# michellelychan/posenet-pytorch

Measured on NVIDIA B200. Metric: images/sec (backbone+decode), higher is better.
Workload: dtype bf16

## Files before the change

posenet-pytorch_b200/csrc/sepconv.cu:

```cuda
#include <cuda.h>
#include <stdlib.h>
#include <string.h>

#include "common.cuh"
#include "ptx.cuh"

namespace pn {

#ifndef PN_SEP_DW_WARPS
#define PN_SEP_DW_WARPS 10
#endif
constexpr int SEP_DW_WARPS = PN_SEP_DW_WARPS;
constexpr int SEP_FIRST_DW_WARP = 6;
constexpr int SEP_THREADS = (SEP_FIRST_DW_WARP + SEP_DW_WARPS) * 32;
constexpr int SEP_MAX_A = 6;
constexpr int SEP_A_BYTES = 128 * 128;
constexpr int SEP_STG_BYTES = 128 * 128;
constexpr int SEP_MAX_P = 6, SEP_MAX_W = 6;
constexpr int SEP_WGT_BYTES = 9 * 64 * 4 + 64 * 4;
constexpr int SEP_SMEM_MAX = 232448;
constexpr int SEP_DWW_KB_BYTES = 10 * 64 * 4;

struct SepGeom {
    int k, nc, ho, wo, pad;
    int th, tw, subs, ths, thi, twi;
    int spr, seg_rows, segs_per_sub;
    unsigned segtab[64];
    int tiles_x, tiles_y, n_tiles, n_tile, panels, tmem_cols;
    int n_halves, n_half, acc_bufs;
    int kblocks;
    int half, cbox;
    int cl;
    int dww_res;
    int w_res;
    unsigned off_dww;
    int teams;
    int exp;
    unsigned epi_sleep_ns;
    int p_stages, w_stages, a_stages, stg_bufs;
    unsigned patch_stage_bytes, patch_box_bytes, wgt_off, w_stage_bytes;
    unsigned off_a, off_stg, off_patch, off_bias, off_bar;
    long long tiles;
};

struct SepBars {
    static constexpr int patch_full = 0, patch_empty = 8 * SEP_MAX_P, w_full = 16 * SEP_MAX_P,
                         w_empty = 16 * SEP_MAX_P + 8 * SEP_MAX_W, a_full = 16 * SEP_MAX_P + 16 * SEP_MAX_W,
                         a_empty = a_full + 8 * SEP_MAX_A, tfull = a_empty + 8 * SEP_MAX_A, tempty = tfull + 16,
                         tmem_slot = tempty + 16, seg_ctr = tmem_slot + 16, seg_tab = seg_ctr + 4 * 8, total = seg_tab + 4 * 64;
};

__device__ __forceinline__ uint64_t sep_smem_desc(uint32_t saddr) {
    return (uint64_t)((saddr & 0x3FFFF) >> 4) | (1ull << 16) | ((uint64_t)(1024 >> 4) << 32) | (1ull << 46) | (2ull << 61);
}
__device__ __forceinline__ uint32_t sep_idesc(int n) {
    return (1u << 4) | (1u << 7) | (1u << 10) | ((uint32_t)(n >> 3) << 17) | ((uint32_t)(128 >> 4) << 24);
}
__device__ __forceinline__ void sep_epi_bar() { asm volatile("bar.sync 1, 128;" ::: "memory"); }
__device__ __forceinline__ float4 lds_f4(uint32_t addr) {
    float4 r;
    asm volatile("ld.shared.v4.f32 {%0, %1, %2, %3}, [%4];" : "=f"(r.x), "=f"(r.y), "=f"(r.z), "=f"(r.w) : "r"(addr));
    return r;
}
__device__ __forceinline__ bool mbar_test(uint32_t bar, uint32_t parity) {
    uint32_t done;
    asm volatile("{\n\t.reg .pred p;\n\tmbarrier.test_wait.parity.shared::cta.b64 p, [%1], %2;\n\tselp.u32 %0, 1, 0, p;\n\t}"
                 : "=r"(done) : "r"(bar), "r"(parity) : "memory");
    return done != 0;
}
__device__ __forceinline__ float2 lds_f2(uint32_t addr) {
    float2 r;
    asm volatile("ld.shared.v2.f32 {%0, %1}, [%2];" : "=f"(r.x), "=f"(r.y) : "r"(addr));
    return r;
}
__device__ __forceinline__ uint32_t lds_u32(uint32_t addr) {
    uint32_t r;
    asm volatile("ld.shared.b32 %0, [%1];" : "=r"(r) : "r"(addr));
    return r;
}
__device__ __forceinline__ uint32_t cluster_rank() {
    uint32_t r;
    asm volatile("mov.u32 %0, %%cluster_ctarank;" : "=r"(r));
    return r;
}
__device__ __forceinline__ void cluster_sync_all() {
    asm volatile("barrier.cluster.arrive.release.aligned;" ::: "memory");
    asm volatile("barrier.cluster.wait.acquire.aligned;" ::: "memory");
}
__device__ __forceinline__ uint32_t map_to_cta(uint32_t saddr, uint32_t rank) {
    uint32_t r;
    asm volatile("mapa.shared::cluster.u32 %0, %1, %2;" : "=r"(r) : "r"(saddr), "r"(rank));
    return r;
}
__device__ __forceinline__ void remote_expect_tx(uint32_t cluster_bar, uint32_t bytes) {
    asm volatile("mbarrier.arrive.expect_tx.release.cluster.shared::cluster.b64 _, [%0], %1;" ::"r"(cluster_bar), "r"(bytes) : "memory");
}
__device__ __forceinline__ void dsmem_bulk_copy(uint32_t cluster_dst, uint32_t src, uint32_t bytes, uint32_t cluster_bar) {
    asm volatile("cp.async.bulk.shared::cluster.shared::cta.mbarrier::complete_tx::bytes [%0], [%1], %2, [%3];" ::"r"(cluster_dst),
                 "r"(src), "r"(bytes), "r"(cluster_bar)
                 : "memory");
}
__device__ __forceinline__ void tc_commit_multicast(uint32_t bar, uint16_t cta_mask) {
    asm volatile("tcgen05.commit.cta_group::1.mbarrier::arrive::one.shared::cluster.multicast::cluster.b64 [%0], %1;" ::"r"(bar),
                 "h"(cta_mask)
                 : "memory");
}
__device__ __forceinline__ void sts_u32_if(uint32_t addr, uint32_t v, bool on) {
    if (on) asm volatile("st.shared.b32 [%0], %1;" ::"r"(addr), "r"(v) : "memory");
}

template <int S, int D, bool HALF> struct SepDwCfg {
    static constexpr bool SLIDE = true;
    static constexpr int RSTEP = (S == 1) ? D : 1;
    static constexpr int DR = (S == 1) ? 1 : D;
    static constexpr bool UNPACKED = (D <= 2);
    static constexpr int NR = 2 * DR + 1;
    static constexpr int HS = HALF ? 2 * S : S;
    static constexpr int NCOLS = 3 * HS + 2 * D + 1;
    static constexpr int PRE = 2 * DR + 1 - S;
};


#ifdef PN_SEP_TRACE
__device__ long long *g_sep_trace = nullptr;
__device__ int g_sep_trace_cap = 0;
#endif
#if defined(PN_SEP_TRACE) && !defined(PN_SEP_PHASES)
#define SEP_TRACE(role, idx, what)                                                                               \
    do {                                                                                                         \
        if (blockIdx.x == 0 && g_sep_trace && (idx) < g_sep_trace_cap)                                           \
            g_sep_trace[((role) * g_sep_trace_cap + (idx)) * 4 + (what)] = clock64();                            \
    } while (0)
#else
#define SEP_TRACE(role, idx, what) do { } while (0)
#endif

// ... 73 lines not shown
    if (DWW_RES) {
        float *sw = reinterpret_cast<float *>(sep_smem_raw + (base - smem_u32(sep_smem_raw)) + g.off_dww);
        for (int i = threadIdx.x; i < g.kblocks * 640; i += SEP_THREADS) {
            const int kbi = i / 640, r = i - kbi * 640, t = r >> 6, ch = kbi * 64 + (r & 63);
            sw[i] = ch < g.k ? (t < 9 ? __ldg(dw_w + (size_t)t * g.k + ch) : __ldg(dw_b + ch)) : 0.f;
        }
    }
    tc_fence_before();
    __syncthreads();
    if (CLUSTER) cluster_sync_all();
    tc_fence_after();
    pdl_launch_dependents();
    pdl_wait();
    const uint32_t tmem_base = *tmem_slot_ptr;

    if (warp == 0) {
        if (lane == 0) {
            int ps = 0, ws = 0, tr_p = 0;
            uint32_t pph = 0, wph = 0;
            (void)tr_p;
            long long p_tile = tile_first, w_tile = tile_first;
            int p_kb = rank, p_sub = 0, w_kb = 0, w_hf = 0;
            int p_img = 0, p_ty = 0, p_tx = 0, w_col = 0;
            bool p_new = true, w_new = true;
            int s_as = rank;
            uint32_t s_aph = 0;
            long long s_left = 0;
            if (CLUSTER && tile_first < g.tiles) s_left = ((g.tiles - tile_first + tile_step - 1) / tile_step) * (g.kblocks / CL);
            const long long t0 = clock64();
            while (p_tile < g.tiles || w_tile < g.tiles || s_left > 0) {
                bool progress = false;
                if (CLUSTER && s_left > 0 && mbar_test(bar(SepBars::a_full, s_as), s_aph)) {
                    const uint32_t sa = a_addr(s_as);
#pragma unroll
                    for (int pr = 0; pr < CL; ++pr)
                        if (pr != rank) {
                            const uint32_t rbar = map_to_cta(bar(SepBars::a_full, s_as), (uint32_t)pr);
                            remote_expect_tx(rbar, SEP_A_BYTES);
                            dsmem_bulk_copy(map_to_cta(sa, (uint32_t)pr), sa, SEP_A_BYTES, rbar);
                        }
                    s_as += CL;
                    if (s_as >= g.a_stages) { s_as -= g.a_stages; s_aph ^= 1; }
                    --s_left;
                    progress = true;
                }
                if (p_tile < g.tiles) {
                    if (p_new) {
                        const int m_tile = (int)(p_tile / g.n_tiles);
                        p_img = m_tile / m_tiles_per_img;
                        const int rem = m_tile - p_img * m_tiles_per_img;
                        p_ty = rem / g.tiles_x;
                        p_tx = rem - p_ty * g.tiles_x;
                        p_new = false;
                    }
                    if (mbar_test(bar(SepBars::patch_empty, ps), pph ^ 1)) {
                        const uint32_t full = bar(SepBars::patch_full, ps);
                        SEP_TRACE(3, tr_p, 0);
#ifdef PN_SEP_EXP
                        if (g.exp & 32) mbar_arrive(full); else {
#endif
                        mbar_expect_tx(full, g.patch_box_bytes + (DWW_RES ? 0u : (uint32_t)SEP_WGT_BYTES));
                        tma_load_4d(p_addr(ps), &tmap_x, full, p_kb * CB, p_tx * g.tw * S - g.pad,
                                    (p_ty * g.th + p_sub * g.ths) * S - g.pad, p_img);
                        if (!DWW_RES) {
                            tma_load_2d(p_addr(ps) + g.wgt_off, &tmap_dww, full, p_kb * CB, 0);
                            tma_load_2d(p_addr(ps) + g.wgt_off + 9 * 64 * 4, &tmap_dwb, full, p_kb * CB, 0);
                        }
#ifdef PN_SEP_EXP
                        }
#endif
                        SEP_TRACE(3, tr_p, 1);
                        ++tr_p;
                        if (++ps == g.p_stages) { ps = 0; pph ^= 1; }
                        if (++p_sub == g.subs) {
                            p_sub = 0;
                            p_kb += CL;
                            if (p_kb >= g.kblocks) { p_kb = rank; p_tile += tile_step; p_new = true; }
                        }
                        progress = true;
                    }
                }
                if (w_tile < g.tiles) {
                    if (w_new) { w_col = col_base + (int)(w_tile % g.n_tiles) * g.n_tile; w_new = false; }
                    if (mbar_test(bar(SepBars::w_empty, ws), wph ^ 1)) {
#ifdef PN_SEP_EXP
                        if (g.exp & 8) mbar_arrive(bar(SepBars::w_full, ws)); else {
#endif
                        mbar_expect_tx(bar(SepBars::w_full, ws), g.w_stage_bytes);
                        tma_load_2d(w_addr(ws), &tmap_w, bar(SepBars::w_full, ws), w_kb * CB, w_col + w_hf * g.n_half);
#ifdef PN_SEP_EXP
                        }
#endif
                        if (++ws == g.w_stages) { ws = 0; wph ^= 1; }
                        if (++w_hf == g.n_halves) {
                            w_hf = 0;
                            if (++w_kb == g.kblocks) {
                                w_kb = 0; w_tile += tile_step; w_new = true;
                                if (g.w_res) w_tile = g.tiles;
                            }
                        }
                        progress = true;
                    }
                }
                if (!progress) {
                    __nanosleep(32);
                    if (clock64() - t0 > 20000000000ll) {
                        printf("posenet_b200: sepconv producer timeout (block %d)\n", blockIdx.x);
                        __trap();
                    }
                }
            }
        }
    } else if (warp == 1) {
        if (lane == 0) {
            const uint32_t idesc = sep_idesc(g.n_half);
            int as = 0, ws = 0, acc = 0, tr_i = 0;
            uint32_t aph = 0, wph = 0, acc_phase = 0;
            (void)tr_i;
            long long kb_total = 0;
            for (long long tile = tile_first; tile < g.tiles; tile += tile_step) {
                mbar_wait(bar(SepBars::tempty, acc), acc_phase ^ 1);
                tc_fence_after();
                SEP_TRACE(1, tr_i, 0);
                const uint32_t d_tmem = tmem_base + (uint32_t)(acc * g.n_tile);
                for (int kb = 0; kb < g.kblocks; ++kb) {
                    mbar_wait(bar(SepBars::a_full, as), aph);
                    SEP_TRACE(1, tr_i, 1);
                    const uint32_t sa = a_addr(as);
                    const int rem_k = g.k - kb * CB;
                    const int ksteps = rem_k >= CB ? CB / 16 : (rem_k + 15) / 16;
                    for (int hf = 0; hf < g.n_halves; ++hf) {
                        if (g.w_res) {
                            ws = kb * g.n_halves + hf;
                            if (tile == tile_first) mbar_wait(bar(SepBars::w_full, ws), 0);
                        } else
                            mbar_wait(bar(SepBars::w_full, ws), wph);
                        tc_fence_after();
                        const uint32_t sb = w_addr(ws);
#pragma unroll
                        for (int k = 0; k < CB / 16; ++k)
                            if (k < ksteps
#ifdef PN_SEP_EXP
                                && !(g.exp & 4)
#endif
                                )
                                tc_mma_bf16(d_tmem + (uint32_t)(hf * g.n_half), sep_smem_desc(sa + k * 32), sep_smem_desc(sb + k * 32), idesc,
                                            (uint32_t)((kb | k) != 0));
                        if (!g.w_res) {
                            tc_commit(bar(SepBars::w_empty, ws));
                            if (++ws == g.w_stages) { ws = 0; wph ^= 1; }
                        }
                    }
                    if (CLUSTER) tc_commit_multicast(bar(SepBars::a_empty, as), (uint16_t)((1u << CL) - 1u));
                    else tc_commit(bar(SepBars::a_empty, as));
                    ++kb_total;
                    SEP_TRACE(1, tr_i, 2);
                    ++tr_i;
                    if (++as == g.a_stages) { as = 0; aph ^= 1; }
                }
                tc_commit(bar(SepBars::tfull, acc));
                if (++acc == g.acc_bufs) { acc = 0; acc_phase ^= 1; }
            }
            if (CLUSTER) {
                for (int s2 = 0; s2 < g.a_stages; ++s2) {
                    if (kb_total <= s2) continue;
                    const long long uses = (kb_total - s2 + g.a_stages - 1) / g.a_stages;
                    mbar_wait(bar(SepBars::a_empty, s2), (uint32_t)((uses - 1) & 1));
                }
            }
        }
    } else if (warp < SEP_FIRST_DW_WARP) {
        const int q = warp & 3;
        const int row_in_tile = q * 32 + lane;
        const bool issuer = (threadIdx.x == 64);
        const uint32_t staging = base + g.off_stg;
        int acc = 0, buf = 0, tr_e = 0;
        uint32_t acc_phase = 0;
        (void)tr_e;
        if (g.stg_bufs == 0) {
            const int r_ty = row_in_tile / g.tw, r_tx = row_in_tile - r_ty * g.tw;
            const int chunks = (g.n_tile + 31) >> 5;
            auto emit = [&](const uint32_t (&v)[32], int c, __nv_bfloat16 *yrow, bool row_ok, int col_lim, uint32_t bias_base) {
                const int col0 = c * 32;
#pragma unroll
                for (int piece = 0; piece < 2; ++piece) {
                    uint32_t o[8];
#pragma unroll
                    for (int j = 0; j < 8; j += 2) {
                        const float4 b0 = lds_f4(bias_base + (uint32_t)(col0 + piece * 16 + j * 2) * 4u);
                        const int i0 = piece * 16 + j * 2;
                        const float2 s0 = fadd2(make_float2(__uint_as_float(v[i0 + 0]), __uint_as_float(v[i0 + 1])), make_float2(b0.x, b0.y));
                        const float2 s1 = fadd2(make_float2(__uint_as_float(v[i0 + 2]), __uint_as_float(v[i0 + 3])), make_float2(b0.z, b0.w));
                        o[j] = relu6_bf16x2(s0);
                        o[j + 1] = relu6_bf16x2(s1);
                    }
                    if (row_ok && col0 + piece * 16 < col_lim)
                        asm volatile("st.global.v8.b32 [%0], {%1, %2, %3, %4, %5, %6, %7, %8};" ::"l"(yrow + col0 + piece * 16), "r"(o[0]),
                                     "r"(o[1]), "r"(o[2]), "r"(o[3]), "r"(o[4]), "r"(o[5]), "r"(o[6]), "r"(o[7])
                                     : "memory");
                }
            };
            for (long long tile = tile_first; tile < g.tiles; tile += tile_step) {
                const int n_tile = (int)(tile % g.n_tiles);
                const int m_tile = (int)(tile / g.n_tiles);
                const int img = m_tile / m_tiles_per_img;
                const int rem = m_tile - img * m_tiles_per_img;
                const int ty = rem / g.tiles_x, tx = rem - ty * g.tiles_x;
                const int oy = ty * g.th + r_ty, ox = tx * g.tw + r_tx;
                bool row_ok = r_ty < g.th && oy < g.ho && ox < g.wo;
#ifdef PN_SEP_EXP
                if (g.exp & 16) row_ok = false;
#endif
                const int colg = col_base + n_tile * g.n_tile;
                __nv_bfloat16 *yrow = y + (((size_t)img * g.ho + oy) * g.wo + ox) * (size_t)g.nc + colg;
                const int col_lim = g.nc - colg;
                mbar_wait_backoff(bar(SepBars::tfull, acc), acc_phase, g.epi_sleep_ns);
                tc_fence_after();
                if (issuer) SEP_TRACE(2, tr_e, 0);
                const uint32_t taddr = tmem_base + ((uint32_t)(q * 32) << 16) + (uint32_t)(acc * g.n_tile);
                const uint32_t bias_base = base + g.off_bias + (uint32_t)(n_tile * g.n_tile) * 4u;
                uint32_t va[32], vb[32];
                tc_ld32(taddr, va);
#pragma unroll 1
                for (int c = 0; c < chunks; c += 2) {
                    tc_ld_wait();
                    if (c + 1 < chunks) tc_ld32(taddr + (uint32_t)((c + 1) * 32), vb);
                    else { tc_fence_before(); mbar_arrive(bar(SepBars::tempty, acc)); }
                    emit(va, c, yrow, row_ok, col_lim, bias_base);
                    if (c + 1 < chunks) {
                        tc_ld_wait();
                        if (c + 2 < chunks) tc_ld32(taddr + (uint32_t)((c + 2) * 32), va);
                        else { tc_fence_before(); mbar_arrive(bar(SepBars::tempty, acc)); }
                        emit(vb, c + 1, yrow, row_ok, col_lim, bias_base);
                    }
                }
                if (issuer) { SEP_TRACE(2, tr_e, 1); ++tr_e; }
                if (++acc == g.acc_bufs) { acc = 0; acc_phase ^= 1; }
            }
        } else
        for (long long tile = tile_first; tile < g.tiles; tile += tile_step) {
            const int n_tile = (int)(tile % g.n_tiles);
            const int m_tile = (int)(tile / g.n_tiles);
            const int img = m_tile / m_tiles_per_img;
            const int rem = m_tile - img * m_tiles_per_img;
            const int ty = rem / g.tiles_x, tx = rem - ty * g.tiles_x;
            mbar_wait_backoff(bar(SepBars::tfull, acc), acc_phase, g.epi_sleep_ns);
            tc_fence_after();
            if (issuer) SEP_TRACE(2, tr_e, 0);
            const uint32_t taddr = tmem_base + ((uint32_t)(q * 32) << 16) + (uint32_t)(acc * g.n_tile);
#ifdef PN_SEP_EXP
            if (g.exp & 2) {
                tc_fence_before();
                mbar_arrive(bar(SepBars::tempty, acc));
                if (++acc == g.acc_bufs) { acc = 0; acc_phase ^= 1; }
                continue;
            }
#endif
#pragma unroll 1
            for (int p = 0; p < g.panels; ++p) {
                const int col0 = n_tile * g.n_tile + p * 64;
                if (issuer) {
                    if (g.stg_bufs == 2) bulk_wait_read<1>(); else bulk_wait_read<0>();
                }
                sep_epi_bar();
                const uint32_t srow = staging + (uint32_t)buf * SEP_STG_BYTES + (uint32_t)row_in_tile * 128u;
#pragma unroll
                for (int hf = 0; hf < 2; ++hf) {
                    uint32_t v[32];
                    tc_ld32(taddr + (uint32_t)(p * 64 + hf * 32), v);
                    tc_ld_wait();
                    if (p == g.panels - 1 && hf == 1) {
                        tc_fence_before();
                        mbar_arrive(bar(SepBars::tempty, acc));
                    }
#pragma unroll
                    for (int c = 0; c < 4; ++c) {
                        const uint32_t bsm = base + g.off_bias + (uint32_t)(col0 + hf * 32 + c * 8) * 4u;
                        const float4 b0 = lds_f4(bsm), b1 = lds_f4(bsm + 16);
                        const float2 s0 = fadd2(make_float2(__uint_as_float(v[8 * c + 0]), __uint_as_float(v[8 * c + 1])), make_float2(b0.x, b0.y));
                        const float2 s1 = fadd2(make_float2(__uint_as_float(v[8 * c + 2]), __uint_as_float(v[8 * c + 3])), make_float2(b0.z, b0.w));
                        const float2 s2 = fadd2(make_float2(__uint_as_float(v[8 * c + 4]), __uint_as_float(v[8 * c + 5])), make_float2(b1.x, b1.y));
                        const float2 s3 = fadd2(make_float2(__uint_as_float(v[8 * c + 6]), __uint_as_float(v[8 * c + 7])), make_float2(b1.z, b1.w));
                        st_shared_v4(srow + (uint32_t)(((hf * 4 + c) ^ (row_in_tile & 7)) << 4), relu6_bf16x2(s0), relu6_bf16x2(s1),
                                     relu6_bf16x2(s2), relu6_bf16x2(s3));
                    }
                }
                fence_async_smem();
                sep_epi_bar();
                if (issuer) {
                    tma_store_4d(&tmap_y, staging + (uint32_t)buf * SEP_STG_BYTES, col_base + col0, tx * g.tw, ty * g.th, img);
                    bulk_commit();
                }
                if (g.stg_bufs == 2) buf ^= 1;
            }
            if (issuer) { SEP_TRACE(2, tr_e, 1); ++tr_e; }
            if (++acc == g.acc_bufs) { acc = 0; acc_phase ^= 1; }
        }
        if (issuer) bulk_wait_all();
    } else {
        using Cfg = SepDwCfg<S, D, HALF>;
        constexpr int NR = Cfg::NR, NCOLS = Cfg::NCOLS, PRE = Cfg::PRE, HS = Cfg::HS, RSTEP = Cfg::RSTEP, DR = Cfg::DR;
        constexpr bool SLIDE = Cfg::SLIDE, UNPACKED = Cfg::UNPACKED, PREFETCH = Cfg::UNPACKED;
        constexpr int NNEW = S;
        constexpr uint32_t PIX = HALF ? 64u : 128u;
        const int hsel = HALF ? (lane >> 4) : 0, cp = HALF ? (lane & 15) : lane;
        const uint32_t rowb1 = (uint32_t)g.twi * PIX, rowb = rowb1 * RSTEP;
        const uint32_t lane_off = (uint32_t)(hsel * S) * PIX + (uint32_t)cp * 4u;
        const uint32_t a_lane = (uint32_t)(cp >> 2) << 4 | (uint32_t)(cp & 3) << 2;
        auto unpack = [](uint32_t r) { return make_float2(__uint_as_float(r << 16), __uint_as_float(r & 0xffff0000u)); };
        const uint32_t tab_addr = bars + (uint32_t)SepBars::seg_tab;

        const int n_teams = g.teams, dwi = warp - SEP_FIRST_DW_WARP, team_max = (SEP_DW_WARPS + n_teams - 1) / n_teams;
        const int big_teams = SEP_DW_WARPS - n_teams * (team_max - 1);
        const int team = dwi < big_teams * team_max ? dwi / team_max : big_teams + (dwi - big_teams * team_max) / (team_max - 1);
        const int team_first = team < big_teams ? team * team_max : big_teams * team_max + (team - big_teams) * (team_max - 1);
        const int team_warps = team < big_teams ? team_max : team_max - 1;
        const bool twice = team_warps < team_max && dwi == team_first;
        const int n_subs = g.subs, n_pst = g.p_stages, n_ast = g.a_stages, n_kb = g.kblocks;
        const int item_step = CLUSTER ? CL : n_teams;
        int tr_d = 0;
// ... 185 lines not shown
#include "sep_tuned.inc"
    {0, 0, 0, 0, 0, 0, 0, 0, 0, 0, 0, 0, 0, 0}};
static int next_pow2_cols(int c) {
    int p = 32;
    while (p < c) p <<= 1;
    return p;
}

bool sep_supported(int k, int nc, int stride, int dil) {
    return k % 8 == 0 && nc % 16 == 0 && k >= 8 && nc >= 16 &&
           ((stride == 1 && (dil == 1 || dil == 2 || dil == 4)) || (stride == 2 && dil == 1));
}

bool sep_fuse_recommended(int k, int nc, int stride, int dil) {
    if (!sep_supported(k, nc, stride, dil)) return false;
    if (nc <= 512) return true;
    return nc == 1024 && k % 64 == 0 && (k / 64) % 4 == 0 && getenv("PN_SEP_CLUSTER") != nullptr;
}

int sep_geometry(SepOp *op, int n, int h, int wd, int k, int nc, int stride, int dil) {
    PN_CHECK_ARG(n > 0 && h > 0 && wd > 0, "pn_sepconv_block: bad shape");
    PN_CHECK_ARG(sep_supported(k, nc, stride, dil), "pn_sepconv_block: unsupported block (cin %d cout %d stride %d dilation %d)", k,
                 nc, stride, dil);
    memset(op, 0, sizeof(*op));
    if (sepwarp_supported(k, nc, stride, dil)) {
        op->warp_kind = true;
        op->stride = stride; op->dil = dil;
        op->ho = (h - 1) / stride + 1; op->wo = (wd - 1) / stride + 1;
        op->n = n; op->h = h; op->w = wd; op->k = k; op->nc = nc;
        return PN_OK;
    }
    if (septc_preferred(k, nc, stride, dil)) {
        op->tc_kind = true;
        op->stride = stride; op->dil = dil;
        op->ho = h; op->wo = wd;
        op->n = n; op->h = h; op->w = wd; op->k = k; op->nc = nc;
        return septc_geometry(&op->tc, n, h, wd, k, nc, dil);
    }
    SepGeom g;
    memset(&g, 0, sizeof(g));
    g.k = k; g.nc = nc;
    g.pad = ((stride - 1) + dil * 2) / 2;
    g.ho = (h + 2 * g.pad - 2 * dil - 1) / stride + 1;
    g.wo = (wd + 2 * g.pad - 2 * dil - 1) / stride + 1;
    PN_CHECK_ARG(g.ho > 0 && g.wo > 0, "pn_sepconv_block: empty output");
    const int cb = 64;
    const bool slide = dil == 1;
    g.half = (k <= 32 && stride == 1 && dil == 1) ? 1 : 0;
    g.cbox = g.half ? 32 : cb;
    const int sw = g.half ? 8 : 4;
    const int ncols = 3 * stride * (g.half ? 2 : 1) + 2 * dil + 1, pre = slide ? 2 * dil + 1 - stride : 0;
    g.kblocks = ceil_div(k, cb);
    g.n_tiles = ceil_div(nc, 512);
    g.n_tile = nc / g.n_tiles;
    g.cl = 1;
    if ((nc == 512 || nc == 1024) && k % cb == 0 && (k / cb) % (nc / 256) == 0 && getenv("PN_SEP_CLUSTER") != nullptr) {
        g.cl = nc / 256;
        g.n_tiles = 1;
        g.n_tile = 256;
    }
    g.n_halves = g.n_tile > 256 ? 2 : 1;
    if (const char *e = getenv("PN_SEP_NBLK")) {
        const int want = atoi(e);
        if (want >= 64 && want % 16 == 0 && g.n_tile > want && g.n_tile % want == 0 && g.n_tile / want <= 4) g.n_halves = g.n_tile / want;
    }
    g.n_half = g.n_tile / g.n_halves;
    PN_CHECK_ARG(g.n_tile * g.n_tiles * g.cl == nc && g.n_half * g.n_halves == g.n_tile && g.n_half % 16 == 0,
                 "pn_sepconv_block: cout %d does not split into tiles", nc);
    g.panels = ceil_div(g.n_tile, 64);
    g.acc_bufs = g.n_tile > 256 ? 1 : 2;
    g.tmem_cols = g.n_tile > 256 ? 512 : next_pow2_cols(g.n_tile + g.panels * 64);
    PN_CHECK_ARG(g.tmem_cols <= 512 && g.panels * 64 <= 512, "pn_sepconv_block: TMEM budget exceeded");
    g.w_stage_bytes = (unsigned)g.n_half * 128u;

    const char *e_dww = getenv("PN_SEP_DWWRES"), *e_wres = getenv("PN_SEP_WRES");
    const bool dww_res = !(e_dww && e_dww[0] == '0') && g.cl == 1 && g.kblocks <= 4;
    const int wgt_stage = dww_res ? 0 : SEP_WGT_BYTES;
    const int dww_bytes = dww_res ? g.kblocks * SEP_DWW_KB_BYTES : 0;
    g.dww_res = dww_res ? 1 : 0;
    g.w_res = (!(e_wres && e_wres[0] == '0') && g.cl == 1 && g.n_tiles == 1 && g.kblocks * g.n_halves <= SEP_MAX_W &&
               (long long)g.kblocks * g.n_halves * g.w_stage_bytes <= 80 * 1024) ? 1 : 0;
    const int min_w = g.w_res ? g.kblocks * g.n_halves : g.n_halves >= 2 ? 3 : 2;
    const int min_a = g.cl > 2 ? g.cl : 2;
    const int fixed = min_a * SEP_A_BYTES + SEP_STG_BYTES + min_w * (int)g.w_stage_bytes + 1024 + 640 + 4224 + dww_bytes;
    double best = 1e300;
    const SepTuned *tuned = nullptr;
    {
        const char *e = getenv("PN_SEP_TUNED");
        if (!(e && e[0] == '0') && g.cl == 1)
            for (const SepTuned &t : SEP_TUNED)
                if (t.k == k && t.nc == nc && t.stride == stride && t.dil == dil && t.ho == g.ho && t.wo == g.wo) { tuned = &t; break; }
    }
    int f_th = 0, f_tw = 0, f_subs = 0;
    if (tuned) { f_th = tuned->th; f_tw = tuned->tw; f_subs = tuned->subs; }
    if (const char *force = getenv("PN_SEP_TILE"))
        if (sscanf(force, "%d,%d,%d", &f_th, &f_tw, &f_subs) != 3) f_th = f_tw = f_subs = 0;
    for (int th = 1; th <= 64; ++th) {
        for (int tw = 1; tw <= 64; ++tw) {
            if (th * tw > 128) break;
            if ((th - 1) >= g.ho + 7 || (tw - 1) >= g.wo + 7) continue;
            for (int subs = 1; subs <= 4 && subs <= th; ++subs) {
                if (f_th && (th != f_th || tw != f_tw || subs != f_subs)) continue;
                const int ths = ceil_div(th, subs);
                if ((subs - 1) * ths >= th) continue;
                const int thi = (ths - 1) * stride + 2 * dil + 1;
                const int twi = (tw - 1) * stride + 2 * dil + 1;
                if (thi > 256 || twi > 256) continue;
                const long long box = (long long)thi * twi * g.cbox * 2;
                const long long stage = ((box + 127) & ~127ll) + wgt_stage;
                const int spr = ceil_div(tw, sw);
                const int rstep = stride == 1 ? dil : 1;
                const int class_rows = ceil_div(ths, rstep);
                int pieces = ceil_div(class_rows, 5);
                if (pieces * spr * subs * rstep < 8) pieces = ceil_div(8, spr * subs * rstep);
                if (pieces > class_rows) pieces = class_rows;
                const int seg_rows = ceil_div(class_rows, pieces);
                int segs = 0;
                for (int c = 0; c < rstep && c < ths; ++c) segs += spr * ceil_div(ceil_div(ths - c, rstep), seg_rows);
                if (segs > 64 || seg_rows > 255 || tw > 255 || ths > 255) continue;
                const long long room = SEP_SMEM_MAX - fixed;
                const int pst = (int)(room / stage);
                if (pst < 2 || pst < subs + 1) continue;
                const long long tiles = (long long)ceil_div(g.ho, th) * ceil_div(g.wo, tw);
                const double step = 45.0 + 10.0 * ncols * (slide ? (stride + 2.0) / 3.0 : 1.0), prol = 1.3 * pre * ncols + 120.0;
                const double lat = 0.5 * (seg_rows * step + prol) * 1.6;
                const double issue = 1.25 * (double)subs * (spr * ths * step + segs * prol) / 4.0;
                const double dwc = lat > issue ? lat : issue;
                const double mma = 2.0 * g.n_tile;
                const double fill = (double)subs * stage / 40.0;
                double per_kb = dwc > mma ? dwc : mma;
                if (fill > per_kb) per_kb = fill;
                per_kb += 0.25 * fill;
                if (pst < 3 * subs) per_kb *= 1.08;
                const double cost = (double)tiles * (g.kblocks * per_kb + 400.0 + 200.0 * g.panels);
                if (cost < best) {
                    best = cost;
                    g.th = th; g.tw = tw; g.subs = subs; g.ths = ths; g.thi = thi; g.twi = twi; g.spr = spr; g.seg_rows = seg_rows;
                    g.segs_per_sub = segs;
                    g.patch_box_bytes = (unsigned)box;
                    g.wgt_off = (unsigned)((box + 127) & ~127ll);
                    g.patch_stage_bytes = (unsigned)stage;
                }
            }
        }
    }
    PN_CHECK_ARG(best < 1e300, "pn_sepconv_block: no tile shape fits (cin %d stride %d dilation %d)", k, stride, dil);
    {
        const int rstep = stride == 1 ? dil : 1;
        int nseg = 0;
        for (int c = 0; c < rstep && c < g.ths; ++c) {
            const int rows_c = ceil_div(g.ths - c, rstep);
            for (int r = 0; r < rows_c; r += g.seg_rows)
                for (int cs = 0; cs < g.spr; ++cs) {
                    const int nrow = rows_c - r < g.seg_rows ? rows_c - r : g.seg_rows;
                    g.segtab[nseg++] = (unsigned)(cs * sw) | (unsigned)(c + r * rstep) << 8 | (unsigned)nrow << 16;
                }
        }
        PN_CHECK_ARG(nseg == g.segs_per_sub, "pn_sepconv_block: internal segment accounting error (%d vs %d)", nseg, g.segs_per_sub);
    }
    g.tiles_x = ceil_div(g.wo, g.tw);
    g.tiles_y = ceil_div(g.ho, g.th);
    g.tiles = (long long)n * g.tiles_x * g.tiles_y * g.n_tiles;
    const long long bias_bytes = ((long long)g.n_tiles * g.panels * 64 * 4 + 127) & ~127ll;
    const long long avail = SEP_SMEM_MAX - 1024 - 640 - bias_bytes - dww_bytes;
    auto fits = [&](int pst, int wst, int ast, int stg) {
        return (long long)wst * g.w_stage_bytes + (long long)ast * SEP_A_BYTES + (long long)stg * SEP_STG_BYTES +
                   (long long)pst * g.patch_stage_bytes <= avail;
    };
    int bestp = -1;
    bool direct = g.acc_bufs == 1 && g.cl == 1;
    if (const char *e = getenv("PN_SEP_DIRECT")) direct = atoi(e) != 0;
    const int max_a1 = direct ? 4 : 3;
    for (int stg = direct ? 0 : 2; stg >= (direct ? 0 : 1); --stg)
        for (int ast = SEP_MAX_A; ast >= 2; --ast) {
            if (g.cl == 1 && ast > max_a1) continue;
            if (g.cl > 1 && ast % g.cl != 0) continue;
            for (int wst = g.w_res ? min_w : SEP_MAX_W; wst >= min_w; --wst)
                for (int pst = SEP_MAX_P; pst >= 2 && pst >= g.subs + 1; --pst) {
                    if (!fits(pst, wst, ast, stg)) continue;
                    const int want = g.cl > 1 ? (g.subs + 1 > 2 ? g.subs + 1 : 2) : 3 * g.subs > SEP_MAX_P ? SEP_MAX_P : 3 * g.subs;
                    const int score = (pst >= want ? 1000 : pst * 100) + (wst > min_w + (direct ? 0 : 1) ? min_w + (direct ? 0 : 1) : wst) * 20 +
                                      (g.cl > 1 ? (ast > 4 ? 4 : ast) * 16 : ast * (direct ? 24 : 8)) + stg * 4 + (pst > want ? 1 : 0);
                    if (score > bestp) {
                        bestp = score;
                        g.p_stages = pst; g.w_stages = wst; g.a_stages = ast; g.stg_bufs = stg;
                    }
                }
        }
    PN_CHECK_ARG(bestp >= 0, "pn_sepconv_block: shared memory budget exceeded");
    if (!direct && g.n_halves == 2 && g.subs == 1 && fits(2, min_w, 3, 2)) { g.p_stages = 2; g.w_stages = min_w; g.a_stages = 3; g.stg_bufs = 2; }
    {
        int fp = 0, fw = 0, fa = 0, fs = 0;
        bool have = false;
        if (tuned && tuned->p > 0 && g.th == tuned->th && g.tw == tuned->tw && g.subs == tuned->subs) { fp = tuned->p; fw = tuned->w; fa = tuned->a; fs = tuned->stg; have = true; }
        if (const char *force = getenv("PN_SEP_STAGES")) have = sscanf(force, "%d,%d,%d,%d", &fp, &fw, &fa, &fs) == 4;
        if (have && fp >= g.subs + 1 && fp <= SEP_MAX_P && fw >= 1 &&
            fw <= SEP_MAX_W && fa >= 2 && fa <= SEP_MAX_A && fa % g.cl == 0 && fs >= 0 && fs <= 2 && fits(fp, fw, fa, fs)) {
            g.p_stages = fp; g.w_stages = fw; g.a_stages = fa; g.stg_bufs = fs;
        }
    }
#ifdef PN_SEP_EXP
    if (const char *e = getenv("PN_SEP_EXP")) g.exp = atoi(e);
#endif
    if (g.w_res && g.w_stages != g.kblocks * g.n_halves) g.w_res = 0;
    g.teams = (g.cl == 1 && SEP_DW_WARPS % 2 == 0 && g.p_stages >= 2 * g.subs + 1 && g.a_stages >= 3 && g.p_stages >= g.a_stages) ? 2 : 1;
    {
        const char *e = getenv("PN_SEP_TEAMS");
        const int v = e ? atoi(e) : (tuned && tuned->p > 0 && g.th == tuned->th && g.tw == tuned->tw && g.subs == tuned->subs) ? tuned->teams : 0;
        if (v == 1 || (v == 2 && g.cl == 1 && SEP_DW_WARPS % 2 == 0 && g.p_stages >= 2 * g.subs && g.a_stages >= 2 && g.p_stages >= g.a_stages)) g.teams = v;
        if (v == 3 && g.cl == 1 && SEP_DW_WARPS >= 6 && g.p_stages >= 3 * g.subs && g.a_stages >= 3 && g.p_stages >= g.a_stages) g.teams = 3;
    }
    g.epi_sleep_ns = 200;
    if (const char *e = getenv("PN_SEP_EPI_SLEEP")) g.epi_sleep_ns = (unsigned)atoi(e);
    static_assert(SepBars::total <= 640, "barrier block exceeds its reserve");
    g.off_a = (unsigned)g.w_stages * g.w_stage_bytes;
    g.off_stg = g.off_a + (unsigned)g.a_stages * SEP_A_BYTES;
    g.off_patch = g.off_stg + (unsigned)g.stg_bufs * SEP_STG_BYTES;
    g.off_bias = g.off_patch + (unsigned)g.p_stages * g.patch_stage_bytes;
    g.off_dww = g.off_bias + (unsigned)bias_bytes;
    g.off_bar = g.off_dww + (unsigned)dww_bytes;
    op->smem_bytes = (int)(g.off_bar + SepBars::total + 1024);
    PN_CHECK_ARG(op->smem_bytes <= SEP_SMEM_MAX, "pn_sepconv_block: internal smem accounting error (%d)", op->smem_bytes);
    static_assert(sizeof(SepGeom) <= sizeof(op->geom), "SepOp::geom too small");
    memcpy(op->geom, &g, sizeof(g));
    op->cb = cb; op->stride = stride; op->dil = dil;
    op->ho = g.ho; op->wo = g.wo;
    op->n = n; op->h = h; op->w = wd; op->k = k; op->nc = nc;
    return PN_OK;
}

int sep_prepare(SepOp *op, const void *x, const float *dw_w, const float *dw_b, const void *pw_w, void *y, int n, int h,
                int wd, int k, int nc, int stride, int dil) {
    PN_CHECK_ARG(x && dw_w && dw_b && pw_w && y, "pn_sepconv_block: null pointer");
    PN_CHECK_ARG(((uintptr_t)x & 15) == 0 && ((uintptr_t)y & 15) == 0 && ((uintptr_t)pw_w & 15) == 0 && ((uintptr_t)dw_w & 15) == 0 &&
                     ((uintptr_t)dw_b & 15) == 0,
                 "pn_sepconv_block: pointers must be 16-byte aligned");
    int rc = sep_geometry(op, n, h, wd, k, nc, stride, dil);
    if (rc != PN_OK) return rc;
    if (op->warp_kind) {
        op->dw_w = dw_w; op->dw_b = dw_b; op->pw_w = pw_w; op->y = y;
        return sepwarp_prepare(&op->warp, x, n, h, wd, k, nc, stride);
    }
    if (op->tc_kind) {
        op->dw_w = dw_w; op->dw_b = dw_b; op->pw_w = pw_w; op->y = y;
        return septc_prepare(&op->tc, x, pw_w, n, h, wd, k, nc, dil);
    }
    op->y = y;
    op->dw_w = dw_w; op->dw_b = dw_b;
    SepGeom g;
    memcpy(&g, op->geom, sizeof(g));
    {
        const uint64_t dims[4] = {(uint64_t)k, (uint64_t)wd, (uint64_t)h, (uint64_t)n};
        const uint64_t strides[3] = {(uint64_t)k * 2, (uint64_t)wd * k * 2, (uint64_t)h * wd * k * 2};
        const uint32_t box[4] = {(uint32_t)g.cbox, (uint32_t)g.twi, (uint32_t)g.thi, 1u};
        if ((rc = encode_tmap(op->tmap_x, x, 2, 4, dims, strides, box, 0)) != PN_OK) return rc;
    }
    {
        const uint64_t dims[2] = {(uint64_t)k, 9};
        const uint64_t strides[1] = {(uint64_t)k * 4};
        const uint32_t box[2] = {64u, 9u};
        if ((rc = encode_tmap(op->tmap_dww, dw_w, 4, 2, dims, strides, box, 0)) != PN_OK) return rc;
        const uint64_t bdims[2] = {(uint64_t)k, 1};
        const uint32_t bbox[2] = {64u, 1u};
        if ((rc = encode_tmap(op->tmap_dwb, dw_b, 4, 2, bdims, strides, bbox, 0)) != PN_OK) return rc;
    }
    {
        const uint64_t dims[2] = {(uint64_t)k, (uint64_t)nc};
        const uint64_t strides[1] = {(uint64_t)k * 2};
        const uint32_t box[2] = {64u, (uint32_t)g.n_half};
        if ((rc = encode_tmap(op->tmap_w, pw_w, 2, 2, dims, strides, box, 3)) != PN_OK) return rc;
    }
    {
        const uint64_t dims[4] = {(uint64_t)nc, (uint64_t)g.wo, (uint64_t)g.ho, (uint64_t)n};
        const uint64_t strides[3] = {(uint64_t)nc * 2, (uint64_t)g.wo * nc * 2, (uint64_t)g.ho * g.wo * nc * 2};
        const uint32_t box[4] = {64u, (uint32_t)g.tw, (uint32_t)g.th, 1u};
        if ((rc = encode_tmap(op->tmap_y, y, 2, 4, dims, strides, box, 3)) != PN_OK) return rc;
    }
    return PN_OK;
}

template <int S, int D, bool HALF, int CL>
static int sep_launch_t(const SepOp *op, const SepGeom &g, const float *pw_bias, cudaStream_t st) {
    static DeviceOnce once, clusters;
    const int dev = current_device();
    auto kern = sepconv_kernel<S, D, HALF, CL>;
    cudaLaunchConfig_t cfg;
    memset(&cfg, 0, sizeof(cfg));
    cudaLaunchAttribute attr[1];
    if (CL > 1) {
        attr[0].id = cudaLaunchAttributeClusterDimension;
        attr[0].val.clusterDim.x = CL; attr[0].val.clusterDim.y = 1; attr[0].val.clusterDim.z = 1;
    } else {
        attr[0].id = cudaLaunchAttributeProgrammaticStreamSerialization;
        attr[0].val.programmaticStreamSerializationAllowed = 1;
    }
    cfg.blockDim = dim3(SEP_THREADS, 1, 1);
    cfg.dynamicSmemBytes = (size_t)op->smem_bytes;
    cfg.stream = st;
    cfg.attrs = attr;
    cfg.numAttrs = (CL > 1 || pdl_enabled()) ? 1 : 0;
    if (!once.get(dev)) {
        PN_CHECK_CUDA(cudaFuncSetAttribute(kern, cudaFuncAttributeMaxDynamicSharedMemorySize, SEP_SMEM_MAX));
        if (CL > 1) {
            int max_clusters = 0;
            cfg.gridDim = dim3((unsigned)(num_sms() / CL * CL), 1, 1);
            cfg.dynamicSmemBytes = SEP_SMEM_MAX;
            PN_CHECK_CUDA(cudaOccupancyMaxActiveClusters(&max_clusters, kern, &cfg));
            PN_CHECK_ARG(max_clusters > 0, "pn_sepconv_block: no %d-CTA cluster fits on this device", CL);
            cfg.dynamicSmemBytes = (size_t)op->smem_bytes;
            clusters.set(dev, max_clusters);
        }
        once.set(dev, 1);
    }
    const long long units = CL > 1 ? clusters.get(dev) : num_sms();
    const int grid = (int)(g.tiles < units ? g.tiles : units) * CL;
    cfg.gridDim = dim3((unsigned)grid, 1, 1);
    PN_CHECK_CUDA(cudaLaunchKernelEx(&cfg, kern, *reinterpret_cast<const CUtensorMap *>(op->tmap_x),
                                     *reinterpret_cast<const CUtensorMap *>(op->tmap_dww), *reinterpret_cast<const CUtensorMap *>(op->tmap_dwb),
                                     *reinterpret_cast<const CUtensorMap *>(op->tmap_w), *reinterpret_cast<const CUtensorMap *>(op->tmap_y),
                                     pw_bias, reinterpret_cast<__nv_bfloat16 *>(op->y), op->dw_w, op->dw_b, g));
    return PN_OK;
}

template <int S, int D>
static int sep_launch_cl(const SepOp *op, const SepGeom &g, const float *pw_bias, cudaStream_t st) {
    if (g.cl == 2) return sep_launch_t<S, D, false, 2>(op, g, pw_bias, st);
    if (g.cl == 4) return sep_launch_t<S, D, false, 4>(op, g, pw_bias, st);
    return sep_launch_t<S, D, false, 1>(op, g, pw_bias, st);
}

int sep_launch(const SepOp *op, const float *pw_bias, cudaStream_t st) {
    PN_CHECK_ARG(op && pw_bias, "pn_sepconv_block: null pointer");
    if (op->warp_kind) return sepwarp_launch(&op->warp, op->dw_w, op->dw_b, op->pw_w, pw_bias, op->y, st);
    if (op->tc_kind) return septc_launch(&op->tc, op->dw_w, op->dw_b, pw_bias, op->y, st);
    SepGeom g;
    memcpy(&g, op->geom, sizeof(g));
    if (op->stride == 2) return sep_launch_cl<2, 1>(op, g, pw_bias, st);
    if (g.half) return sep_launch_t<1, 1, true, 1>(op, g, pw_bias, st);
    if (op->dil == 1) return sep_launch_cl<1, 1>(op, g, pw_bias, st);
    if (op->dil == 2) return sep_launch_cl<1, 2>(op, g, pw_bias, st);
    return sep_launch_cl<1, 4>(op, g, pw_bias, st);
}

void sep_describe(const SepOp *op, char *out, size_t cap) {
    if (op->tc_kind) {
        septc_describe(&op->tc, out, cap);
        return;
    }
    if (op->warp_kind) {
        SepWarpOp w;
        if (sepwarp_geometry(&w, op->n, op->h, op->w, op->k, op->nc, op->stride) == PN_OK) sepwarp_describe(&w, out, cap);
        else snprintf(out, cap, "warp-autonomous (geometry unavailable)");
        return;
    }
    SepGeom g;
    memcpy(&g, op->geom, sizeof(g));
    snprintf(out, cap, "%s%stile %dx%d subs %d box %dx%d segs %d x %d rows n_tile %d(%dx%d) x%d kblocks %d teams %d stages p%d w%d%s a%d stg%d smem %d tiles %lld",
             g.half ? "half " : "", g.cl == 2 ? "cluster2 " : g.cl == 4 ? "cluster4 " : "", g.th, g.tw, g.subs, g.thi, g.twi, g.segs_per_sub, g.seg_rows, g.n_tile, g.n_halves, g.n_half, g.n_tiles, g.kblocks, g.teams, g.p_stages,
             g.w_stages, g.w_res ? "r" : "", g.a_stages, g.stg_bufs, op->smem_bytes, g.tiles);
}

}

#ifdef PN_SEP_TRACE
extern "C" int pn_debug_sep_trace(long long *buf, int cap) {
    if (cudaMemcpyToSymbol(pn::g_sep_trace, &buf, sizeof(buf)) != cudaSuccess) return -2;
    if (cudaMemcpyToSymbol(pn::g_sep_trace_cap, &cap, sizeof(cap)) != cudaSuccess) return -2;
    return 0;
}
#endif
```

Before: 42830.

## Add A-resident lagged two-half MMA schedule for stride-2 separable convs

```diff
diff --git a/posenet-pytorch_b200/csrc/sepconv.cu b/posenet-pytorch_b200/csrc/sepconv.cu
--- a/posenet-pytorch_b200/csrc/sepconv.cu
+++ b/posenet-pytorch_b200/csrc/sepconv.cu
@@ -13,7 +13,7 @@
 constexpr int SEP_DW_WARPS = PN_SEP_DW_WARPS;
 constexpr int SEP_FIRST_DW_WARP = 6;
 constexpr int SEP_THREADS = (SEP_FIRST_DW_WARP + SEP_DW_WARPS) * 32;
-constexpr int SEP_MAX_A = 6;
+constexpr int SEP_MAX_A = 8;
 constexpr int SEP_A_BYTES = 128 * 128;
 constexpr int SEP_STG_BYTES = 128 * 128;
 constexpr int SEP_MAX_P = 6, SEP_MAX_W = 6;
@@ -34,6 +34,7 @@
     int dww_res;
     int w_res;
     unsigned off_dww;
+    int ares, lag;
     int teams;
     int exp;
     unsigned epi_sleep_ns;
@@ -52,6 +53,15 @@
 
 __device__ __forceinline__ uint64_t sep_smem_desc(uint32_t saddr) {
     return (uint64_t)((saddr & 0x3FFFF) >> 4) | (1ull << 16) | ((uint64_t)(1024 >> 4) << 32) | (1ull << 46) | (2ull << 61);
+}
+__device__ __forceinline__ uint64_t sep_smem_desc_sw64(uint32_t saddr) {
+    return (uint64_t)((saddr & 0x3FFFF) >> 4) | (1ull << 16) | ((uint64_t)(512 >> 4) << 32) | (1ull << 46) | (4ull << 61);
+}
+__device__ __forceinline__ void sep_ares_op(int j, int kbs, int lag, int &hf, int &kb) {
+    if (j < lag) { hf = 0; kb = j; return; }
+    j -= lag;
+    if (j < 2 * (kbs - lag)) { hf = (j & 1) ? 0 : 1; kb = (j >> 1) + ((j & 1) ? lag : 0); return; }
+    hf = 1; kb = kbs - lag + (j - 2 * (kbs - lag));
 }
 __device__ __forceinline__ uint32_t sep_idesc(int n) {
     return (1u << 4) | (1u << 7) | (1u << 10) | ((uint32_t)(n >> 3) << 17) | ((uint32_t)(128 >> 4) << 24);
@@ -291,7 +301,18 @@
                 }
                 if (w_tile < g.tiles) {
                     if (w_new) { w_col = col_base + (int)(w_tile % g.n_tiles) * g.n_tile; w_new = false; }
-                    if (mbar_test(bar(SepBars::w_empty, ws), wph ^ 1)) {
+                    if (g.ares && mbar_test(bar(SepBars::w_empty, ws), wph ^ 1)) {
+                        int hf, kb;
+                        sep_ares_op(w_kb, g.kblocks, g.lag, hf, kb);
+                        mbar_expect_tx(bar(SepBars::w_full, ws), g.w_stage_bytes);
+                        tma_load_2d(w_addr(ws), &tmap_w, bar(SepBars::w_full, ws), kb * CB + w_hf * (CB / 2), w_col + hf * g.n_half);
+                        if (++ws == g.w_stages) { ws = 0; wph ^= 1; }
+                        if (++w_hf == 2) {
+                            w_hf = 0;
+                            if (++w_kb == 2 * g.kblocks) { w_kb = 0; w_tile += tile_step; w_new = true; }
+                        }
+                        progress = true;
+                    } else if (!g.ares && mbar_test(bar(SepBars::w_empty, ws), wph ^ 1)) {
 #ifdef PN_SEP_EXP
                         if (g.exp & 8) mbar_arrive(bar(SepBars::w_full, ws)); else {
 #endif
@@ -327,6 +348,53 @@
             uint32_t aph = 0, wph = 0, acc_phase = 0;
             (void)tr_i;
             long long kb_total = 0;
+            if (g.ares) {
+                uint32_t tph = 0;
+                int as1 = 0;
+                for (long long tile = tile_first; tile < g.tiles; tile += tile_step) {
+                    SEP_TRACE(1, tr_i, 0);
+                    for (int j = 0; j < 2 * g.kblocks; ++j) {
+                        int hf, kb;
+                        sep_ares_op(j, g.kblocks, g.lag, hf, kb);
+                        if (kb == 0) {
+                            mbar_wait(bar(SepBars::tempty, hf), tph ^ 1);
+                            tc_fence_after();
+                        }
+                        const int sidx = hf == 0 ? as : as1;
+                        if (hf == 0) {
+                            mbar_wait(bar(SepBars::a_full, as), aph);
+                            if (++as == g.a_stages) { as = 0; aph ^= 1; }
+                        }
+                        SEP_TRACE(1, tr_i, 1);
+                        const uint32_t sa = a_addr(sidx), d_tmem = tmem_base + (uint32_t)(hf * g.n_half);
+                        const int rem_k = g.k - kb * CB;
+                        const int ksteps = rem_k >= CB ? CB / 16 : (rem_k + 15) / 16;
+#pragma unroll
+                        for (int kh = 0; kh < 2; ++kh) {
+                            mbar_wait(bar(SepBars::w_full, ws), wph);
+                            tc_fence_after();
+                            const uint32_t sb = w_addr(ws);
+#pragma unroll
+                            for (int kk = 0; kk < 2; ++kk) {
+                                const int k = 2 * kh + kk;
+                                if (k < ksteps)
+                                    tc_mma_bf16(d_tmem, sep_smem_desc(sa + k * 32), sep_smem_desc_sw64(sb + kk * 32), idesc,
+                                                (uint32_t)((kb | k) != 0));
+                            }
+                            tc_commit(bar(SepBars::w_empty, ws));
+                            if (++ws == g.w_stages) { ws = 0; wph ^= 1; }
+                        }
+                        if (hf == 1) {
+                            tc_commit(bar(SepBars::a_empty, as1));
+                            if (++as1 == g.a_stages) as1 = 0;
+                        }
+                        if (kb == g.kblocks - 1) tc_commit(bar(SepBars::tfull, hf));
+                        SEP_TRACE(1, tr_i, 2);
+                        ++tr_i;
+                    }
+                    tph ^= 1;
+                }
+            } else
             for (long long tile = tile_first; tile < g.tiles; tile += tile_step) {
                 mbar_wait(bar(SepBars::tempty, acc), acc_phase ^ 1);
                 tc_fence_after();
@@ -388,7 +456,8 @@
         (void)tr_e;
         if (g.stg_bufs == 0) {
             const int r_ty = row_in_tile / g.tw, r_tx = row_in_tile - r_ty * g.tw;
-            const int chunks = (g.n_tile + 31) >> 5;
+            const int units = g.ares ? 2 : 1, ucols = g.n_tile / units;
+            const int chunks = (ucols + 31) >> 5;
             auto emit = [&](const uint32_t (&v)[32], int c, __nv_bfloat16 *yrow, bool row_ok, int col_lim, uint32_t bias_base) {
                 const int col0 = c * 32;
 #pragma unroll
@@ -420,14 +489,17 @@
 #ifdef PN_SEP_EXP
                 if (g.exp & 16) row_ok = false;
 #endif
-                const int colg = col_base + n_tile * g.n_tile;
+#pragma unroll 1
+                for (int u = 0; u < units; ++u) {
+                const int colt = n_tile * g.n_tile + u * ucols;
+                const int colg = col_base + colt;
                 __nv_bfloat16 *yrow = y + (((size_t)img * g.ho + oy) * g.wo + ox) * (size_t)g.nc + colg;
                 const int col_lim = g.nc - colg;
                 mbar_wait_backoff(bar(SepBars::tfull, acc), acc_phase, g.epi_sleep_ns);
                 tc_fence_after();
                 if (issuer) SEP_TRACE(2, tr_e, 0);
-                const uint32_t taddr = tmem_base + ((uint32_t)(q * 32) << 16) + (uint32_t)(acc * g.n_tile);
-                const uint32_t bias_base = base + g.off_bias + (uint32_t)(n_tile * g.n_tile) * 4u;
+                const uint32_t taddr = tmem_base + ((uint32_t)(q * 32) << 16) + (uint32_t)(acc * ucols);
+                const uint32_t bias_base = base + g.off_bias + (uint32_t)colt * 4u;
                 uint32_t va[32], vb[32];
                 tc_ld32(taddr, va);
 #pragma unroll 1
@@ -445,6 +517,7 @@
                 }
                 if (issuer) { SEP_TRACE(2, tr_e, 1); ++tr_e; }
                 if (++acc == g.acc_bufs) { acc = 0; acc_phase ^= 1; }
+                }
             }
         } else
         for (long long tile = tile_first; tile < g.tiles; tile += tile_step) {
@@ -796,7 +869,7 @@
                (long long)g.kblocks * g.n_halves * g.w_stage_bytes <= 80 * 1024) ? 1 : 0;
     const int min_w = g.w_res ? g.kblocks * g.n_halves : g.n_halves >= 2 ? 3 : 2;
     const int min_a = g.cl > 2 ? g.cl : 2;
-    const int fixed = min_a * SEP_A_BYTES + SEP_STG_BYTES + min_w * (int)g.w_stage_bytes + 1024 + 640 + 4224 + dww_bytes;
+    const int fixed = min_a * SEP_A_BYTES + SEP_STG_BYTES + min_w * (int)g.w_stage_bytes + 1024 + SepBars::total + 4224 + dww_bytes;
     double best = 1e300;
     const SepTuned *tuned = nullptr;
     {
@@ -876,7 +949,7 @@
     g.tiles_y = ceil_div(g.ho, g.th);
     g.tiles = (long long)n * g.tiles_x * g.tiles_y * g.n_tiles;
     const long long bias_bytes = ((long long)g.n_tiles * g.panels * 64 * 4 + 127) & ~127ll;
-    const long long avail = SEP_SMEM_MAX - 1024 - 640 - bias_bytes - dww_bytes;
+    const long long avail = SEP_SMEM_MAX - 1024 - SepBars::total - bias_bytes - dww_bytes;
     auto fits = [&](int pst, int wst, int ast, int stg) {
         return (long long)wst * g.w_stage_bytes + (long long)ast * SEP_A_BYTES + (long long)stg * SEP_STG_BYTES +
                    (long long)pst * g.patch_stage_bytes <= avail;
@@ -903,7 +976,33 @@
         }
     PN_CHECK_ARG(bestp >= 0, "pn_sepconv_block: shared memory budget exceeded");
     if (!direct && g.n_halves == 2 && g.subs == 1 && fits(2, min_w, 3, 2)) { g.p_stages = 2; g.w_stages = min_w; g.a_stages = 3; g.stg_bufs = 2; }
-    {
+    const char *e_ares = getenv("PN_SEP_ARES");
+    const bool ares_want = e_ares ? e_ares[0] == '1' : stride == 2;
+    if (ares_want && direct && g.cl == 1 && g.n_tiles == 1 && g.n_halves == 2 && g.n_half % 32 == 0 && g.kblocks >= 2 && g.kblocks <= SEP_MAX_A) {
+        const unsigned ring_w_bytes = g.w_stage_bytes;
+        g.w_stage_bytes = (unsigned)g.n_half * 64u;
+        int pst = 0;
+        for (int p = SEP_MAX_P; p >= g.subs + 1 && !pst; --p)
+            if (p % (2 * g.subs) == 0 && fits(p, 3, g.kblocks, 0)) pst = p;
+        for (int p = SEP_MAX_P; p >= g.subs + 1 && !pst; --p)
+            if (fits(p, 3, g.kblocks, 0)) pst = p;
+        if (pst) {
+            int wst = 3;
+            while (wst < SEP_MAX_W && fits(pst, wst + 1, g.kblocks, 0)) ++wst;
+            g.ares = 1; g.acc_bufs = 2; g.w_res = 0;
+            g.p_stages = pst; g.w_stages = wst; g.a_stages = g.kblocks; g.stg_bufs = 0;
+            int fp = 0, fw = 0, fa = 0, fs = 0;
+            if (const char *force = getenv("PN_SEP_STAGES"))
+                if (sscanf(force, "%d,%d,%d,%d", &fp, &fw, &fa, &fs) == 4 && fp >= g.subs + 1 && fp <= SEP_MAX_P && fw >= 2 &&
+                    fw <= SEP_MAX_W && fa >= 2 && fa <= g.kblocks && fs == 0 && fits(fp, fw, fa, 0)) {
+                    g.p_stages = fp; g.w_stages = fw; g.a_stages = fa;
+                }
+            g.lag = g.a_stages / 2;
+            if (const char *e = getenv("PN_SEP_LAG")) { const int l = atoi(e); if (l >= 1 && l <= g.a_stages) g.lag = l; }
+        } else
+            g.w_stage_bytes = ring_w_bytes;
+    }
+    if (!g.ares) {
         int fp = 0, fw = 0, fa = 0, fs = 0;
         bool have = false;
         if (tuned && tuned->p > 0 && g.th == tuned->th && g.tw == tuned->tw && g.subs == tuned->subs) { fp = tuned->p; fw = tuned->w; fa = tuned->a; fs = tuned->stg; have = true; }
@@ -924,9 +1023,14 @@
         if (v == 1 || (v == 2 && g.cl == 1 && SEP_DW_WARPS % 2 == 0 && g.p_stages >= 2 * g.subs && g.a_stages >= 2 && g.p_stages >= g.a_stages)) g.teams = v;
         if (v == 3 && g.cl == 1 && SEP_DW_WARPS >= 6 && g.p_stages >= 3 * g.subs && g.a_stages >= 3 && g.p_stages >= g.a_stages) g.teams = 3;
     }
+    if (g.ares) {
+        const char *e = getenv("PN_SEP_TEAMS");
+        const bool own = g.a_stages % 2 == 0 && g.p_stages % (2 * g.subs) == 0;
+        const bool deep = g.p_stages >= 2 * g.subs + 1 && g.a_stages >= 3 && g.p_stages >= g.a_stages;
+        g.teams = (SEP_DW_WARPS % 2 == 0 && (own || deep) && !(e && atoi(e) == 1)) ? 2 : 1;
+    }
     g.epi_sleep_ns = 200;
     if (const char *e = getenv("PN_SEP_EPI_SLEEP")) g.epi_sleep_ns = (unsigned)atoi(e);
-    static_assert(SepBars::total <= 640, "barrier block exceeds its reserve");
     g.off_a = (unsigned)g.w_stages * g.w_stage_bytes;
     g.off_stg = g.off_a + (unsigned)g.a_stages * SEP_A_BYTES;
     g.off_patch = g.off_stg + (unsigned)g.stg_bufs * SEP_STG_BYTES;
@@ -981,8 +1085,8 @@
     {
         const uint64_t dims[2] = {(uint64_t)k, (uint64_t)nc};
         const uint64_t strides[1] = {(uint64_t)k * 2};
-        const uint32_t box[2] = {64u, (uint32_t)g.n_half};
-        if ((rc = encode_tmap(op->tmap_w, pw_w, 2, 2, dims, strides, box, 3)) != PN_OK) return rc;
+        const uint32_t box[2] = {g.ares ? 32u : 64u, (uint32_t)g.n_half};
+        if ((rc = encode_tmap(op->tmap_w, pw_w, 2, 2, dims, strides, box, g.ares ? 2 : 3)) != PN_OK) return rc;
     }
     {
         const uint64_t dims[4] = {(uint64_t)nc, (uint64_t)g.wo, (uint64_t)g.ho, (uint64_t)n};
@@ -1069,8 +1173,10 @@
     }
     SepGeom g;
     memcpy(&g, op->geom, sizeof(g));
-    snprintf(out, cap, "%s%stile %dx%d subs %d box %dx%d segs %d x %d rows n_tile %d(%dx%d) x%d kblocks %d teams %d stages p%d w%d%s a%d stg%d smem %d tiles %lld",
-             g.half ? "half " : "", g.cl == 2 ? "cluster2 " : g.cl == 4 ? "cluster4 " : "", g.th, g.tw, g.subs, g.thi, g.twi, g.segs_per_sub, g.seg_rows, g.n_tile, g.n_halves, g.n_half, g.n_tiles, g.kblocks, g.teams, g.p_stages,
+    char mode[24] = "";
+    if (g.ares) snprintf(mode, sizeof(mode), "ares L%d ", g.lag);
+    snprintf(out, cap, "%s%s%stile %dx%d subs %d box %dx%d segs %d x %d rows n_tile %d(%dx%d) x%d kblocks %d teams %d stages p%d w%d%s a%d stg%d smem %d tiles %lld",
+             g.half ? "half " : "", g.cl == 2 ? "cluster2 " : g.cl == 4 ? "cluster4 " : "", mode, g.th, g.tw, g.subs, g.thi, g.twi, g.segs_per_sub, g.seg_rows, g.n_tile, g.n_halves, g.n_half, g.n_tiles, g.kblocks, g.teams, g.p_stages,
              g.w_stages, g.w_res ? "r" : "", g.a_stages, g.stg_bufs, op->smem_bytes, g.tiles);
 }
 
```

Measured after the change: 42900 (median of 6 runs). No clear change (+0.2%).
